# caoql98/LKGD

Measured on AMD Instinct MI355X. Metric: denoised frames/sec (14f x 576x1024, 25-step Euler), higher is better.
Workload: dtype f16; 1 GPU; SVD 14 frames x 576x1024, 25 Euler steps, CFG 1.0->3.0, single clip, vanilla pipeline_stable_video_diffusion_trans loop (configs[1]); unet=random-init SVD shapes (320,640,1280,1280), heads (5,10,20,20), 1.52 B params, parallelism=single GPU

## Files before the change

lkgd_amd/csrc/norm.hip:

```cpp
#include "common.h"
#include "../../include/lkgd_hip_dit.h"

static thread_local int gn_apply_kb = 32;
extern "C" void lkgd_debug_set_gn_apply_kb(int kb) { gn_apply_kb = kb < 32 ? 32 : kb; }
static thread_local int gn_stats_kb = 128;
extern "C" void lkgd_debug_set_gn_stats_kb(int kb) { gn_stats_kb = kb < 32 ? 32 : kb; }
static thread_local int gn_target_wgs = 1024;
extern "C" void lkgd_debug_set_gn_target_wgs(int n) { gn_target_wgs = n < 1 ? 1 : n; }
static inline int gn_rows_kb(int C, int kb, long long rows_per_sample, long long nsamples) {
  int rmax = kb * 1024 / (C * 2);
  rmax = rmax < 8 ? 8 : (rmax > 1024 ? 1024 : rmax);
  int rmin = 8 * 1024 / (C * 2);
  rmin = rmin < 8 ? 8 : rmin;
  if (rmin > rmax) rmin = rmax;
  const long long want = (rows_per_sample * nsamples + gn_target_wgs - 1) / gn_target_wgs;
  return (int)(want < rmin ? rmin : (want > rmax ? rmax : want));
}
static inline int gn_rows(int C, long long rows_per_sample, long long nsamples) {
  return gn_rows_kb(C, gn_apply_kb, rows_per_sample, nsamples);
}
static inline int gn_rows_stats(int C, long long rows_per_sample, long long nsamples) {
  return gn_rows_kb(C, gn_stats_kb, rows_per_sample, nsamples);
}
#define GN_GROUPS 32
#define GN_MAXC 4096

struct GnMap {
  int C8, rows_par, nslot;
};
__device__ __forceinline__ GnMap gn_map(int C) {
  GnMap m;
  m.C8 = C >> 3;
  if (m.C8 <= 256) { m.rows_par = 256 / m.C8; m.nslot = 1; }
  else { m.rows_par = 1; m.nslot = (m.C8 + 255) / 256; }
  return m;
}

__device__ __forceinline__ half8_t gn_load(const half_t* x0, int c0, int ld0, const half_t* x1, int ld1,
                                            long long row, int cv) {
  int c = cv << 3;
  if (c < c0) return *(const half8_t*)(x0 + row * ld0 + c);
  return *(const half8_t*)(x1 + row * ld1 + (c - c0));
}

__global__ __launch_bounds__(256) void gn_stats_kernel(const half_t* x0, int c0, int ld0, const half_t* x1, int c1,
                                                       int ld1, long long rows_per_sample, float* partial,
                                                       int nchunks, int GN_ROWS) {
  __shared__ float s_sum[GN_MAXC];
  __shared__ float s_sq[GN_MAXC];
  const int C = c0 + c1;
  const GnMap mp = gn_map(C);
  const int t = threadIdx.x;
  const int chunk = blockIdx.x;
  const long long sample = blockIdx.y;
  const long long r0 = (long long)chunk * GN_ROWS;
  long long r1 = r0 + GN_ROWS;
  if (r1 > rows_per_sample) r1 = rows_per_sample;
  const long long base = sample * rows_per_sample;
  for (int slot = 0; slot < mp.nslot; ++slot) {
    int cv, rp;
    if (mp.nslot == 1) { rp = t / mp.C8; cv = t - rp * mp.C8; if (rp >= mp.rows_par) continue; }
    else { rp = 0; cv = t + 256 * slot; if (cv >= mp.C8) continue; }
    float s[8], q[8];
#pragma unroll
    for (int e = 0; e < 8; ++e) { s[e] = 0.f; q[e] = 0.f; }
#pragma unroll 8
    for (long long r = r0 + rp; r < r1; r += mp.rows_par) {
      half8_t v = gn_load(x0, c0, ld0, x1, ld1, base + r, cv);
#pragma unroll
      for (int e = 0; e < 8; ++e) { float f = (float)v[e]; s[e] += f; q[e] += f * f; }
    }
#pragma unroll
    for (int e = 0; e < 8; ++e) {
      s_sum[rp * C + cv * 8 + e] = s[e];
      s_sq[rp * C + cv * 8 + e] = q[e];
    }
  }
  __syncthreads();
  if (t < GN_GROUPS) {
    const int gs = C / GN_GROUPS;
    float a = 0.f, b = 0.f;
    for (int rp = 0; rp < mp.rows_par; ++rp)
      for (int c = t * gs; c < (t + 1) * gs; ++c) { a += s_sum[rp * C + c]; b += s_sq[rp * C + c]; }
    float* o = partial + ((sample * nchunks + chunk) * GN_GROUPS + t) * 2;
    o[0] = a; o[1] = b;
  }
}

__device__ __forceinline__ void gn_reduce_pair(const float* partial, int nchunks, long long sample, int g, int lane,
                                               double& sa, double& sb) {
  double a = 0.0, b = 0.0;
  for (int c = lane; c < nchunks; c += 64) {
    const float* p = partial + ((sample * nchunks + c) * GN_GROUPS + g) * 2;
    a += p[0]; b += p[1];
  }
#pragma unroll
  for (int o = 32; o > 0; o >>= 1) { a += __shfl_xor(a, o, 64); b += __shfl_xor(b, o, 64); }
  sa = a; sb = b;
}

__global__ __launch_bounds__(256) void gn_finalize_kernel(const float* partial, int nchunks, double inv_count,
                                                          float eps, float* stats) {
  const int lane = threadIdx.x & 63;
  const int g = blockIdx.x * 4 + (threadIdx.x >> 6);
  const long long sample = blockIdx.y;
  double sa, sb;
  gn_reduce_pair(partial, nchunks, sample, g, lane, sa, sb);
  if (lane == 0) {
    double mean = sa * inv_count;
    double var = sb * inv_count - mean * mean;
    if (var < 0.0) var = 0.0;
    stats[(sample * GN_GROUPS + g) * 2 + 0] = (float)mean;
    stats[(sample * GN_GROUPS + g) * 2 + 1] = (float)(1.0 / sqrt(var + (double)eps));
  }
}

__global__ __launch_bounds__(256) void gn_cols_kernel(const float* cs0, int blk0, int ld0, int c0, const float* cs1, int blk1,
                                                      int ld1, int c1, long long rows_per_sample, double inv_count, float eps,
                                                      int as_sums, float* stats) {
  __shared__ double sa[256], sb[256];
  const int t = threadIdx.x;
  const int g = blockIdx.x;
  const long long sample = blockIdx.y;
  const int gs = (c0 + c1) / GN_GROUPS;
  double a = 0.0, b = 0.0;
  for (int src = 0; src < 2; ++src) {
    const float* cs = src ? cs1 : cs0;
    if (!cs) continue;
    const int blk = src ? blk1 : blk0, ld = src ? ld1 : ld0;
    int lo = g * gs - (src ? c0 : 0), hi = lo + gs;
    const int cmax = src ? c1 : c0;
    lo = lo < 0 ? 0 : lo;
    hi = hi > cmax ? cmax : hi;
    const int nch = hi - lo;
    if (nch <= 0) continue;
    const int plo = lo >> 1, npair = nch >> 1;
    const long long nb = rows_per_sample / blk, b0 = sample * nb;
    const long long total = nb * npair;
    for (long long e = t; e < total; e += 256) {
      const long long bi = e / npair;
      const int c = plo + (int)(e - bi * npair);
      const float* q = cs + ((b0 + bi) * (ld >> 1) + c) * 2;
      a += q[0]; b += q[1];
    }
  }
  sa[t] = a; sb[t] = b;
  __syncthreads();
#pragma unroll
  for (int o = 128; o > 0; o >>= 1) {
    if (t < o) { sa[t] += sa[t + o]; sb[t] += sb[t + o]; }
    __syncthreads();
  }
  if (t == 0) {
    float* o = stats + (sample * GN_GROUPS + g) * 2;
    if (as_sums) {
      o[0] = (float)sa[0]; o[1] = (float)sb[0];
    } else {
      const double mean = sa[0] * inv_count;
      double var = sb[0] * inv_count - mean * mean;
      if (var < 0.0) var = 0.0;
      o[0] = (float)mean;
      o[1] = (float)(1.0 / sqrt(var + (double)eps));
    }
  }
}

__global__ __launch_bounds__(256) void gn_sums_kernel(const float* partial, int nchunks, float* sums) {
  const int lane = threadIdx.x & 63;
  const int g = blockIdx.x * 4 + (threadIdx.x >> 6);
  const long long sample = blockIdx.y;
  double sa, sb;
  gn_reduce_pair(partial, nchunks, sample, g, lane, sa, sb);
  if (lane == 0) {
    sums[(sample * GN_GROUPS + g) * 2 + 0] = (float)sa;
    sums[(sample * GN_GROUPS + g) * 2 + 1] = (float)sb;
  }
}
__global__ void gn_finalize_sums_kernel(const float* sums, long long n, double inv_count, float eps, float* stats) {
  long long i = (long long)blockIdx.x * blockDim.x + threadIdx.x;
  if (i >= n) return;
  double mean = (double)sums[i * 2] * inv_count;
  double var = (double)sums[i * 2 + 1] * inv_count - mean * mean;
  if (var < 0.0) var = 0.0;
  stats[i * 2] = (float)mean;
  stats[i * 2 + 1] = (float)(1.0 / sqrt(var + (double)eps));
}

__global__ __launch_bounds__(256) void gn_apply_kernel(const half_t* x0, int c0, int ld0, const half_t* x1, int c1,
                                                       int ld1, long long rows_per_sample, const float* stats,
                                                       const float* gamma, const float* beta, int silu,
                                                       half_t* out, int ldo, int GN_ROWS) {
  const int C = c0 + c1;
  const GnMap mp = gn_map(C);
  const int t = threadIdx.x;
  const long long sample = blockIdx.y;
  const long long r0 = (long long)blockIdx.x * GN_ROWS;
  long long r1 = r0 + GN_ROWS;
  if (r1 > rows_per_sample) r1 = rows_per_sample;
  const long long base = sample * rows_per_sample;
  const int gs = C / GN_GROUPS;
  for (int slot = 0; slot < mp.nslot; ++slot) {
    int cv, rp;
    if (mp.nslot == 1) { rp = t / mp.C8; cv = t - rp * mp.C8; if (rp >= mp.rows_par) continue; }
    else { rp = 0; cv = t + 256 * slot; if (cv >= mp.C8) continue; }
    float A[8], B[8];
    {
      const float4_t g0 = *(const float4_t*)(gamma + cv * 8), g1 = *(const float4_t*)(gamma + cv * 8 + 4);
      const float4_t b0 = *(const float4_t*)(beta + cv * 8), b1 = *(const float4_t*)(beta + cv * 8 + 4);
      typedef float float2_t __attribute__((ext_vector_type(2)));
#pragma unroll
      for (int e = 0; e < 8; ++e) {
        const int g = (cv * 8 + e) / gs;
        const float2_t mr = *(const float2_t*)(stats + (sample * GN_GROUPS + g) * 2);
        const float ga = e < 4 ? g0[e & 3] : g1[e & 3], be = e < 4 ? b0[e & 3] : b1[e & 3];
        A[e] = mr[1] * ga;
        B[e] = be - mr[0] * A[e];
      }
    }
#pragma unroll 4
    for (long long r = r0 + rp; r < r1; r += mp.rows_par) {
      half8_t v = gn_load(x0, c0, ld0, x1, ld1, base + r, cv);
      half8_t o;
#pragma unroll
      for (int e = 0; e < 8; ++e) {
        float f = (float)v[e] * A[e] + B[e];
        if (silu) f = silu_f(f);
        o[e] = (half_t)f;
      }
      *(half8_t*)(out + (base + r) * ldo + cv * 8) = o;
    }
  }
}

static int gn_check(const void* x0, int c0, int ld0, const void* x1, int c1, int ld1, long long nsamples,
                    long long rows) {
  if (!x0) return LKGD_E_NULL;
  if (c1 > 0 && !x1) return LKGD_E_NULL;
  int C = c0 + c1;
  if (c0 <= 0 || c1 < 0 || C % GN_GROUPS || C % 8 || c0 % 8 || C > GN_MAXC) return LKGD_E_SHAPE;
  if (ld0 % 8 || (c1 > 0 && ld1 % 8)) return LKGD_E_ALIGN;
  if (!aligned16(x0) || (x1 && !aligned16(x1))) return LKGD_E_ALIGN;
  if (nsamples <= 0 || rows <= 0 || nsamples > 65535) return LKGD_E_SHAPE;
  return LKGD_OK;
}

extern "C" int lkgd_groupnorm_chunks(int64_t rows_per_sample, int32_t C) {
  const int ra = gn_rows(C, rows_per_sample, 1), rs = gn_rows_stats(C, rows_per_sample, 1);
  const int r = ra < rs ? ra : rs;
  return (int)((rows_per_sample + r - 1) / r);
}

extern "C" int lkgd_groupnorm_stats(const void* x0, int32_t c0, int32_t ld0, const void* x1, int32_t c1, int32_t ld1,
                                    int64_t nsamples, int64_t rows_per_sample, float eps, float* partial,
                                    float* stats, lkgd_stream_t stream) {
  int rc = gn_check(x0, c0, ld0, x1, c1, ld1, nsamples, rows_per_sample);
  if (rc) return rc;
  if (!partial || !stats) return LKGD_E_NULL;
  const int rs = gn_rows_stats(c0 + c1, rows_per_sample, nsamples);
  int nchunks = (int)((rows_per_sample + rs - 1) / rs);
  hipLaunchKernelGGL(gn_stats_kernel, dim3(nchunks, (unsigned)nsamples), dim3(256), 0, (hipStream_t)stream,
                     (const half_t*)x0, c0, ld0, (const half_t*)x1, c1, ld1, (long long)rows_per_sample, partial,
                     nchunks, rs);
  double inv = 1.0 / ((double)rows_per_sample * (double)((c0 + c1) / GN_GROUPS));
  hipLaunchKernelGGL(gn_finalize_kernel, dim3(8, (unsigned)nsamples), dim3(256), 0, (hipStream_t)stream, partial,
                     nchunks, inv, eps, stats);
  return hipGetLastError() == hipSuccess ? LKGD_OK : LKGD_E_LAUNCH;
}

extern "C" int lkgd_groupnorm_stats_cols(const float* cs0, int32_t blk0, int32_t ldcs0, int32_t c0, const float* cs1,
                                         int32_t blk1, int32_t ldcs1, int32_t c1, int64_t nsamples, int64_t rows_per_sample,
                                         float eps, int32_t as_sums, float* stats, lkgd_stream_t stream) {
  if (!cs0 || !stats || (c1 > 0 && !cs1)) return LKGD_E_NULL;
  const int C = c0 + c1;
  if ((C / GN_GROUPS) % 2 || c0 % 2 || c1 % 2 || ldcs0 % 2 || ldcs1 % 2) return LKGD_E_SHAPE;
  if (c0 <= 0 || c1 < 0 || C % GN_GROUPS || blk0 <= 0 || ldcs0 < c0 || (c1 > 0 && (blk1 <= 0 || ldcs1 < c1))) return LKGD_E_SHAPE;
  if (nsamples <= 0 || nsamples > 65535 || rows_per_sample <= 0 || rows_per_sample % blk0 || (c1 > 0 && rows_per_sample % blk1))
    return LKGD_E_SHAPE;
  const double inv = 1.0 / ((double)rows_per_sample * (double)(C / GN_GROUPS));
  hipLaunchKernelGGL(gn_cols_kernel, dim3(GN_GROUPS, (unsigned)nsamples), dim3(256), 0, (hipStream_t)stream, cs0, blk0, ldcs0,
                     c0, c1 > 0 ? cs1 : (const float*)nullptr, blk1, ldcs1, c1, (long long)rows_per_sample, inv, eps, as_sums,
                     stats);
  return hipGetLastError() == hipSuccess ? LKGD_OK : LKGD_E_LAUNCH;
}

extern "C" int lkgd_groupnorm_sums(const void* x0, int32_t c0, int32_t ld0, const void* x1, int32_t c1, int32_t ld1,
                                   int64_t nsamples, int64_t rows_per_sample, float* partial, float* sums,
                                   lkgd_stream_t stream) {
  int rc = gn_check(x0, c0, ld0, x1, c1, ld1, nsamples, rows_per_sample);
  if (rc) return rc;
  if (!partial || !sums) return LKGD_E_NULL;
  const int rs = gn_rows_stats(c0 + c1, rows_per_sample, nsamples);
  int nchunks = (int)((rows_per_sample + rs - 1) / rs);
  hipLaunchKernelGGL(gn_stats_kernel, dim3(nchunks, (unsigned)nsamples), dim3(256), 0, (hipStream_t)stream,
                     (const half_t*)x0, c0, ld0, (const half_t*)x1, c1, ld1, (long long)rows_per_sample, partial,
                     nchunks, rs);
  hipLaunchKernelGGL(gn_sums_kernel, dim3(8, (unsigned)nsamples), dim3(256), 0, (hipStream_t)stream, partial, nchunks,
                     sums);
  return hipGetLastError() == hipSuccess ? LKGD_OK : LKGD_E_LAUNCH;
}

__global__ void gn_finalize_parts_kernel(const float* parts, int nparts, long long part_stride, long long sample_stride,
                                         long long n, double inv_count, float eps, float* stats) {
  long long i = (long long)blockIdx.x * blockDim.x + threadIdx.x;
  if (i >= n) return;
  const long long sample = i / GN_GROUPS;
  const int g = (int)(i - sample * GN_GROUPS);
  double a = 0.0, b = 0.0;
  for (int r = 0; r < nparts; ++r) {
    const float* p = parts + r * part_stride + sample * sample_stride + g * 2;
    a += (double)p[0]; b += (double)p[1];
  }
  double mean = a * inv_count;
  double var = b * inv_count - mean * mean;
  if (var < 0.0) var = 0.0;
  stats[i * 2] = (float)mean;
  stats[i * 2 + 1] = (float)(1.0 / sqrt(var + (double)eps));
}

extern "C" int lkgd_groupnorm_finalize_parts(const float* parts, int32_t nparts, int64_t part_stride, int64_t nsamples,
                                             int64_t sample_stride, double count_per_group, float eps, float* stats,
                                             lkgd_stream_t stream) {
  if (!parts || !stats) return LKGD_E_NULL;
  if (nparts <= 0 || nsamples <= 0 || part_stride < 0 || sample_stride < GN_GROUPS * 2 || !(count_per_group > 0.0)) return LKGD_E_SHAPE;
  if (((uintptr_t)parts & 3u) != 0) return LKGD_E_ALIGN;
  long long n = nsamples * GN_GROUPS;
  hipLaunchKernelGGL(gn_finalize_parts_kernel, dim3((unsigned)((n + 255) / 256)), dim3(256), 0, (hipStream_t)stream, parts,
                     nparts, (long long)part_stride, (long long)sample_stride, n, 1.0 / count_per_group, eps, stats);
  return hipGetLastError() == hipSuccess ? LKGD_OK : LKGD_E_LAUNCH;
}

extern "C" int lkgd_groupnorm_finalize(const float* sums, int64_t nsamples, double count_per_group, float eps,
                                       float* stats, lkgd_stream_t stream) {
  if (!sums || !stats) return LKGD_E_NULL;
  if (nsamples <= 0 || !(count_per_group > 0.0)) return LKGD_E_SHAPE;
  long long n = nsamples * GN_GROUPS;
  hipLaunchKernelGGL(gn_finalize_sums_kernel, dim3((unsigned)((n + 255) / 256)), dim3(256), 0, (hipStream_t)stream,
                     sums, n, 1.0 / count_per_group, eps, stats);
  return hipGetLastError() == hipSuccess ? LKGD_OK : LKGD_E_LAUNCH;
}

extern "C" int lkgd_groupnorm_apply(const void* x0, int32_t c0, int32_t ld0, const void* x1, int32_t c1, int32_t ld1,
                                    int64_t nsamples, int64_t rows_per_sample, const float* stats,
                                    const float* gamma, const float* beta, int32_t silu, void* out, int32_t ldo,
                                    lkgd_stream_t stream) {
  int rc = gn_check(x0, c0, ld0, x1, c1, ld1, nsamples, rows_per_sample);
  if (rc) return rc;
  if (!stats || !gamma || !beta || !out) return LKGD_E_NULL;
  if (ldo % 8 || !aligned16(out)) return LKGD_E_ALIGN;
  const int ra = gn_rows(c0 + c1, rows_per_sample, nsamples);
  int nchunks = (int)((rows_per_sample + ra - 1) / ra);
  hipLaunchKernelGGL(gn_apply_kernel, dim3(nchunks, (unsigned)nsamples), dim3(256), 0, (hipStream_t)stream,
                     (const half_t*)x0, c0, ld0, (const half_t*)x1, c1, ld1, (long long)rows_per_sample, stats, gamma,
                     beta, silu, (half_t*)out, ldo, ra);
  return hipGetLastError() == hipSuccess ? LKGD_OK : LKGD_E_LAUNCH;
}

struct gn_segment { const half_t* src; half_t* dst; long long rows; long long sample; };
__global__ __launch_bounds__(256) void gn_apply_segments_kernel(const gn_segment* segs, int C, int ld, const float* stats,
                                                                const float* gamma, const float* beta, int silu, int GN_ROWS) {
  const gn_segment sg = segs[blockIdx.y];
  const long long r0 = (long long)blockIdx.x * GN_ROWS;
  if (r0 >= sg.rows) return;
  long long r1 = r0 + GN_ROWS;
  if (r1 > sg.rows) r1 = sg.rows;
  const GnMap mp = gn_map(C);
  const int t = threadIdx.x;
  const int gs = C / GN_GROUPS;
  for (int slot = 0; slot < mp.nslot; ++slot) {
    int cv, rp;
    if (mp.nslot == 1) { rp = t / mp.C8; cv = t - rp * mp.C8; if (rp >= mp.rows_par) continue; }
    else { rp = 0; cv = t + 256 * slot; if (cv >= mp.C8) continue; }
    float A[8], B[8];
    {
      const float4_t g0 = *(const float4_t*)(gamma + cv * 8), g1 = *(const float4_t*)(gamma + cv * 8 + 4);
      const float4_t b0 = *(const float4_t*)(beta + cv * 8), b1 = *(const float4_t*)(beta + cv * 8 + 4);
      typedef float float2_t __attribute__((ext_vector_type(2)));
#pragma unroll
      for (int e = 0; e < 8; ++e) {
        const int g = (cv * 8 + e) / gs;
        const float2_t mr = *(const float2_t*)(stats + (sg.sample * GN_GROUPS + g) * 2);
        const float ga = e < 4 ? g0[e & 3] : g1[e & 3], be = e < 4 ? b0[e & 3] : b1[e & 3];
        A[e] = mr[1] * ga;
        B[e] = be - mr[0] * A[e];
      }
    }
#pragma unroll 4
    for (long long r = r0 + rp; r < r1; r += mp.rows_par) {
      const half8_t v = *(const half8_t*)(sg.src + r * ld + cv * 8);
      half8_t o;
#pragma unroll
      for (int e = 0; e < 8; ++e) {
        float f = (float)v[e] * A[e] + B[e];
        if (silu) f = silu_f(f);
        o[e] = (half_t)f;
      }
      *(half8_t*)(sg.dst + r * ld + cv * 8) = o;
    }
  }
}

extern "C" int lkgd_groupnorm_apply_segments(const void* segs, int32_t nseg, int64_t max_rows, int32_t C, int32_t ld,
                                             const float* stats, const float* gamma, const float* beta, int32_t silu,
                                             lkgd_stream_t stream) {
  if (!segs || !stats || !gamma || !beta) return LKGD_E_NULL;
  if (nseg <= 0 || nseg > 65535 || max_rows <= 0 || C <= 0 || C % GN_GROUPS || C % 8 || C > GN_MAXC || ld % 8 || ld < C) return LKGD_E_SHAPE;
  if (((uintptr_t)segs & 7u) != 0) return LKGD_E_ALIGN;
  const int ra = gn_rows(C, max_rows, nseg);
  const int nchunks = (int)((max_rows + ra - 1) / ra);
  hipLaunchKernelGGL(gn_apply_segments_kernel, dim3(nchunks, (unsigned)nseg), dim3(256), 0, (hipStream_t)stream,
                     (const gn_segment*)segs, C, ld, stats, gamma, beta, silu, ra);
  return hipGetLastError() == hipSuccess ? LKGD_OK : LKGD_E_LAUNCH;
}

#define GN_SMALL_NT 512
#define GN_SMALL_U 4
template <int VEC>
__global__ __launch_bounds__(GN_SMALL_NT) void gn_small_kernel(const half_t* x0, int c0, int ld0, const half_t* x1, int c1, int ld1,
                                                               int rows, float eps, const float* gamma, const float* beta, int silu,
                                                               half_t* out, int ldo, float* stats) {
  typedef half_t hv_t __attribute__((ext_vector_type(VEC)));
  extern __shared__ __attribute__((aligned(16))) char gn_smem[];
  hv_t* buf = (hv_t*)gn_smem;
  __shared__ double red[2 * (GN_SMALL_NT / 64)];
  __shared__ float mr[2];
  const int t = threadIdx.x, lane = t & 63, w = t >> 6;
  const int g = blockIdx.x;
  const long long sample = blockIdx.y;
  const int gs = (c0 + c1) / GN_GROUPS, per = gs / VEC;
  const int units = rows * per;
  const long long base = sample * rows;
  const int q = GN_SMALL_NT / per, rem = GN_SMALL_NT - q * per;
  int r = t / per, a = t - r * per;
  float s = 0.f, ss = 0.f;
  for (int u = t; u < units; u += GN_SMALL_NT * GN_SMALL_U) {
    hv_t v[GN_SMALL_U];
#pragma unroll
    for (int k = 0; k < GN_SMALL_U; ++k) {
      const int c = g * gs + a * VEC;
      const bool ok = u + k * GN_SMALL_NT < units;
      const long long row = ok ? base + r : base;
      const half_t* src = c < c0 ? x0 + row * ld0 + c : x1 + row * ld1 + (c - c0);
      v[k] = *(const hv_t*)src;
      r += q; a += rem;
      if (a >= per) { a -= per; ++r; }
    }
#pragma unroll
    for (int k = 0; k < GN_SMALL_U; ++k) {
      if (u + k * GN_SMALL_NT < units) {
        buf[u + k * GN_SMALL_NT] = v[k];
#pragma unroll
        for (int e = 0; e < VEC; ++e) { const float f = (float)v[k][e]; s += f; ss += f * f; }
      }
    }
  }
#pragma unroll
  for (int o = 32; o > 0; o >>= 1) { s += __shfl_xor(s, o, 64); ss += __shfl_xor(ss, o, 64); }
  if (lane == 0) { red[w] = (double)s; red[GN_SMALL_NT / 64 + w] = (double)ss; }
  __syncthreads();
  if (t == 0) {
    const double inv = 1.0 / ((double)rows * (double)gs);
    double sa = 0.0, sb = 0.0;
#pragma unroll
    for (int i = 0; i < GN_SMALL_NT / 64; ++i) { sa += red[i]; sb += red[GN_SMALL_NT / 64 + i]; }
    const double mean = sa * inv;
    double var = sb * inv - mean * mean;
    if (var < 0.0) var = 0.0;
    mr[0] = (float)mean;
    mr[1] = (float)(1.0 / sqrt(var + (double)eps));
    if (stats) { stats[(sample * GN_GROUPS + g) * 2] = mr[0]; stats[(sample * GN_GROUPS + g) * 2 + 1] = mr[1]; }
  }
  __syncthreads();
  const float mean = mr[0], rstd = mr[1];
  r = t / per; a = t - r * per;
  for (int u = t; u < units; u += GN_SMALL_NT) {
    const int c = g * gs + a * VEC;
    const hv_t v = buf[u];
    hv_t o;
#pragma unroll
    for (int e = 0; e < VEC; ++e) {
      const float A = rstd * gamma[c + e], B = beta[c + e] - mean * A;
      float f = (float)v[e] * A + B;
      if (silu) f = silu_f(f);
      o[e] = (half_t)f;
    }
    *(hv_t*)(out + (base + r) * ldo + c) = o;
    r += q; a += rem;
    if (a >= per) { a -= per; ++r; }
  }
}

static thread_local int gn_small_on = 1;
extern "C" void lkgd_debug_set_gn_small(int on) { gn_small_on = on != 0; }
#define GN_SMALL_LDS (48 * 1024)
static thread_local long long gn_small_max_bytes = 10LL * 1024 * 1024 + 512 * 1024;
extern "C" void lkgd_debug_set_gn_small_limits(int64_t total_bytes) { gn_small_max_bytes = total_bytes; }
static int gn_small_vec(int c0, int c1, int ld0, int ld1, int ldo, long long nsamples, long long rows, const void* out) {
  const int C = c0 + c1, gs = C / GN_GROUPS;
  if (!gn_small_on || rows * gs * 2 > GN_SMALL_LDS || nsamples * rows * C * 2 > gn_small_max_bytes || nsamples * GN_GROUPS < 64)
    return 0;
  const int vec = gs % 8 == 0 ? 8 : (gs % 4 == 0 ? 4 : (gs % 2 == 0 ? 2 : 0));
  if (!vec || gs / vec > GN_SMALL_NT || c0 % vec || ld0 % vec || (c1 > 0 && ld1 % vec) || ldo % vec) return 0;
  if (((uintptr_t)out) % (2 * vec)) return 0;
  return vec;
}

extern "C" int lkgd_groupnorm_silu(const void* x0, int32_t c0, int32_t ld0, const void* x1, int32_t c1, int32_t ld1,
                                   int64_t nsamples, int64_t rows_per_sample, float eps, float* partial, float* stats,
                                   const float* gamma, const float* beta, int32_t silu, void* out, int32_t ldo,
                                   lkgd_stream_t stream) {
  const int vec = gn_small_vec(c0, c1, ld0, ld1, ldo, nsamples, rows_per_sample, out);
  if (vec) {
    int rc = gn_check(x0, c0, ld0, x1, c1, ld1, nsamples, rows_per_sample);
    if (rc) return rc;
    if (!gamma || !beta || !out) return LKGD_E_NULL;
    LKGD_DEVICE_ONCE_BEGIN
      if (hipFuncSetAttribute((const void*)gn_small_kernel<8>, hipFuncAttributeMaxDynamicSharedMemorySize, GN_SMALL_LDS) != hipSuccess ||
          hipFuncSetAttribute((const void*)gn_small_kernel<4>, hipFuncAttributeMaxDynamicSharedMemorySize, GN_SMALL_LDS) != hipSuccess ||
          hipFuncSetAttribute((const void*)gn_small_kernel<2>, hipFuncAttributeMaxDynamicSharedMemorySize, GN_SMALL_LDS) != hipSuccess)
        return LKGD_E_LAUNCH;
    LKGD_DEVICE_ONCE_END
    const size_t lds = (size_t)rows_per_sample * ((c0 + c1) / GN_GROUPS) * 2;
    const dim3 grid(GN_GROUPS, (unsigned)nsamples);
#define GN_SMALL_GO(V)                                                                                                   \
  hipLaunchKernelGGL(gn_small_kernel<V>, grid, dim3(GN_SMALL_NT), lds, (hipStream_t)stream, (const half_t*)x0, c0, ld0,          \
                     (const half_t*)x1, c1, ld1, (int)rows_per_sample, eps, gamma, beta, silu, (half_t*)out, ldo, stats)
    if (vec == 8) GN_SMALL_GO(8); else if (vec == 4) GN_SMALL_GO(4); else GN_SMALL_GO(2);
#undef GN_SMALL_GO
    return hipGetLastError() == hipSuccess ? LKGD_OK : LKGD_E_LAUNCH;
  }
  int rc = lkgd_groupnorm_stats(x0, c0, ld0, x1, c1, ld1, nsamples, rows_per_sample, eps, partial, stats, stream);
  if (rc) return rc;
  return lkgd_groupnorm_apply(x0, c0, ld0, x1, c1, ld1, nsamples, rows_per_sample, stats, gamma, beta, silu, out, ldo, stream);
}

#define LN_MAXV 3
#define LN_MAXV_WIDE 4
#define LN_MAXV_XWIDE 6
template <int L, bool AFF, int NV = LN_MAXV>
__global__ __launch_bounds__(256) void layernorm_kernel(const half_t* x, int ldx, long long T, int C,
                                                        const float* gamma, const float* beta, float eps,
                                                        const half_t* rowbias, int ldrb, int d1, int m1, int d2,
                                                        int md, int c0, half_t* out, int ldo) {
  constexpr int RPW = 64 / L;
  const int lane = threadIdx.x & 63;
  const int wave = threadIdx.x >> 6;
  const int sub = lane / L, li = lane % L;
  const int C8 = C >> 3;
  float g[AFF ? NV : 1][8], b[AFF ? NV : 1][8];
  if (AFF) {
#pragma unroll
    for (int v = 0; v < NV; ++v) {
      int cv = li + L * v;
      if (cv >= C8) cv = C8 - 1;
      const float4_t g0 = *(const float4_t*)(gamma + cv * 8), g1 = *(const float4_t*)(gamma + cv * 8 + 4);
      const float4_t b0 = *(const float4_t*)(beta + cv * 8), b1 = *(const float4_t*)(beta + cv * 8 + 4);
#pragma unroll
      for (int e = 0; e < 8; ++e) {
        g[AFF ? v : 0][e] = e < 4 ? g0[e & 3] : g1[e & 3];
        b[AFF ? v : 0][e] = e < 4 ? b0[e & 3] : b1[e & 3];
      }
    }
  }
  const float invC = 1.0f / (float)C;
  const long long rows_per_block = 4 * RPW;
  for (long long row0 = (long long)blockIdx.x * rows_per_block + wave * RPW; row0 < T;
       row0 += (long long)gridDim.x * rows_per_block) {
    const long long row = row0 + sub;
    const bool live = row < T;
    float xv[NV][8];
    float s = 0.f;
    long long idx = 0;
    if (rowbias && live) {
      if (T < (1LL << 31)) {
        const unsigned ru = (unsigned)row;
        idx = ((ru / (unsigned)d1) * (unsigned)m1 + (ru % (unsigned)d2) + (unsigned)c0) % (unsigned)md;
      } else {
        idx = ((row / d1) * m1 + (row % d2) + c0) % md;
      }
    }
#pragma unroll
    for (int v = 0; v < NV; ++v) {
      int cv = li + L * v;
      if (live && cv < C8) {
        half8_t h = *(const half8_t*)(x + row * ldx + cv * 8);
        if (rowbias) {
          half8_t rb = *(const half8_t*)(rowbias + idx * ldrb + cv * 8);
          h = h + rb;
        }
#pragma unroll
        for (int e = 0; e < 8; ++e) { xv[v][e] = (float)h[e]; s += xv[v][e]; }
      } else {
#pragma unroll
        for (int e = 0; e < 8; ++e) xv[v][e] = 0.f;
      }
    }
#pragma unroll
    for (int o = L / 2; o > 0; o >>= 1) s += __shfl_xor(s, o, 64);
    const float mean = s * invC;
    float q = 0.f;
#pragma unroll
    for (int v = 0; v < NV; ++v) {
      int cv = li + L * v;
      if (cv < C8) {
#pragma unroll
        for (int e = 0; e < 8; ++e) { float d = xv[v][e] - mean; q += d * d; }
      }
    }
#pragma unroll
    for (int o = L / 2; o > 0; o >>= 1) q += __shfl_xor(q, o, 64);
    const float rstd = rsqrtf(q * invC + eps);
#pragma unroll
    for (int v = 0; v < NV; ++v) {
      int cv = li + L * v;
      if (live && cv < C8) {
        half8_t o;
#pragma unroll
        for (int e = 0; e < 8; ++e) {
          float y = (xv[v][e] - mean) * rstd;
          if (AFF) y = y * g[AFF ? v : 0][e] + b[AFF ? v : 0][e];
          o[e] = (half_t)y;
        }
        *(half8_t*)(out + row * ldo + cv * 8) = o;
      }
    }
  }
}

extern "C" int lkgd_layernorm(const void* x, int32_t ldx, int64_t T, int32_t C, const float* gamma,
                              const float* beta, float eps, const void* rowbias, int32_t ldrb, int32_t rb_d1,
                              int32_t rb_m1, int32_t rb_d2, int32_t rb_md, void* out, int32_t ldo,
                              lkgd_stream_t stream) {
  if (!x || !out) return LKGD_E_NULL;
  if ((gamma == nullptr) != (beta == nullptr)) return LKGD_E_NULL;
  if (T <= 0 || C <= 0 || C % 8 || C > 64 * 8 * LN_MAXV_XWIDE) return LKGD_E_SHAPE;
  if (ldx % 8 || ldo % 8 || !aligned16(x) || !aligned16(out)) return LKGD_E_ALIGN;
  if (rowbias && (ldrb % 8 || !aligned16(rowbias) || rb_d1 <= 0 || rb_d2 <= 0 || rb_md <= 0)) return LKGD_E_SHAPE;
  const int C8 = C / 8;
  int L = 4;
  while (L < 64 && L * LN_MAXV < C8) L *= 2;
  const long long rows_per_block = 4 * (64 / L);
  long long blocks = (T + rows_per_block - 1) / rows_per_block;
  if (blocks > 256 * 16) blocks = 256 * 16;
#define LN_LAUNCH(LL)                                                                                            \
  if (gamma)                                                                                                     \
    hipLaunchKernelGGL((layernorm_kernel<LL, true>), dim3((unsigned)blocks), dim3(256), 0, (hipStream_t)stream,  \
                       (const half_t*)x, ldx, (long long)T, C, gamma, beta, eps, (const half_t*)rowbias, ldrb,   \
                       rb_d1, rb_m1, rb_d2, rb_md, 0, (half_t*)out, ldo);                                        \
  else                                                                                                           \
    hipLaunchKernelGGL((layernorm_kernel<LL, false>), dim3((unsigned)blocks), dim3(256), 0, (hipStream_t)stream, \
                       (const half_t*)x, ldx, (long long)T, C, gamma, beta, eps, (const half_t*)rowbias, ldrb,   \
                       rb_d1, rb_m1, rb_d2, rb_md, 0, (half_t*)out, ldo)
  if (C8 > 64 * LN_MAXV_WIDE) {
    if (gamma)
      hipLaunchKernelGGL((layernorm_kernel<64, true, LN_MAXV_XWIDE>), dim3((unsigned)blocks), dim3(256), 0, (hipStream_t)stream,
                         (const half_t*)x, ldx, (long long)T, C, gamma, beta, eps, (const half_t*)rowbias, ldrb, rb_d1, rb_m1,
                         rb_d2, rb_md, 0, (half_t*)out, ldo);
    else
      hipLaunchKernelGGL((layernorm_kernel<64, false, LN_MAXV_XWIDE>), dim3((unsigned)blocks), dim3(256), 0, (hipStream_t)stream,
                         (const half_t*)x, ldx, (long long)T, C, gamma, beta, eps, (const half_t*)rowbias, ldrb, rb_d1, rb_m1,
                         rb_d2, rb_md, 0, (half_t*)out, ldo);
    return hipGetLastError() == hipSuccess ? LKGD_OK : LKGD_E_LAUNCH;
  }
  if (C8 > 64 * LN_MAXV) {
    if (gamma)
      hipLaunchKernelGGL((layernorm_kernel<64, true, LN_MAXV_WIDE>), dim3((unsigned)blocks), dim3(256), 0, (hipStream_t)stream,
                         (const half_t*)x, ldx, (long long)T, C, gamma, beta, eps, (const half_t*)rowbias, ldrb, rb_d1, rb_m1,
                         rb_d2, rb_md, 0, (half_t*)out, ldo);
    else
      hipLaunchKernelGGL((layernorm_kernel<64, false, LN_MAXV_WIDE>), dim3((unsigned)blocks), dim3(256), 0, (hipStream_t)stream,
                         (const half_t*)x, ldx, (long long)T, C, gamma, beta, eps, (const half_t*)rowbias, ldrb, rb_d1, rb_m1,
                         rb_d2, rb_md, 0, (half_t*)out, ldo);
    return hipGetLastError() == hipSuccess ? LKGD_OK : LKGD_E_LAUNCH;
  }
  switch (L) {
    case 4: LN_LAUNCH(4); break;
    case 8: LN_LAUNCH(8); break;
    case 16: LN_LAUNCH(16); break;
    case 32: LN_LAUNCH(32); break;
    default: LN_LAUNCH(64); break;
  }
#undef LN_LAUNCH
  return hipGetLastError() == hipSuccess ? LKGD_OK : LKGD_E_LAUNCH;
}

__device__ __forceinline__ half8_t qk_rope8(half8_t x, const float* __restrict__ cs, const float* __restrict__ sn) {
#pragma clang fp contract(off)
  half8_t y;
#pragma unroll
  for (int i = 0; i < 4; ++i) {
    const float a = (float)x[2 * i], b = (float)x[2 * i + 1];
    const float pa = a * cs[2 * i], pb = b * sn[2 * i];
    const float qa = b * cs[2 * i + 1], qb = a * sn[2 * i + 1];
    y[2 * i] = (half_t)(pa - pb);
    y[2 * i + 1] = (half_t)(qa + qb);
  }
  return y;
}

__device__ __forceinline__ void qk_norm_rope_head(half_t* __restrict__ p, bool live, const half8_t (&hv)[2],
                                                  const float (&g)[2][8], const float (&b)[2][8], float eps, bool rot,
                                                  const float (&cs)[2][8], const float (&sn)[2][8]) {
  const float invC = 1.0f / 64.0f;
  float xv[2][8];
  float s = 0.f;
#pragma unroll
  for (int v = 0; v < 2; ++v) {
    if (live) {
#pragma unroll
      for (int e = 0; e < 8; ++e) { xv[v][e] = (float)hv[v][e]; s += xv[v][e]; }
    } else {
#pragma unroll
      for (int e = 0; e < 8; ++e) xv[v][e] = 0.f;
    }
  }
#pragma unroll
  for (int o = 2; o > 0; o >>= 1) s += __shfl_xor(s, o, 64);
  const float mean = s * invC;
  float q = 0.f;
#pragma unroll
  for (int v = 0; v < 2; ++v) {
#pragma unroll
    for (int e = 0; e < 8; ++e) { float d = xv[v][e] - mean; q += d * d; }
  }
#pragma unroll
  for (int o = 2; o > 0; o >>= 1) q += __shfl_xor(q, o, 64);
  const float rstd = rsqrtf(q * invC + eps);
#pragma unroll
  for (int v = 0; v < 2; ++v) {
    if (live) {
      half8_t o;
#pragma unroll
      for (int e = 0; e < 8; ++e) {
        float y = (xv[v][e] - mean) * rstd;
        y = y * g[v][e] + b[v][e];
        o[e] = (half_t)y;
      }
      if (rot) o = qk_rope8(o, cs[v], sn[v]);
      *(half8_t*)(p + 32 * v) = o;
    }
  }
}

__global__ __launch_bounds__(256) void qk_norm_rope_kernel(half_t* q, int ldq, half_t* k, int ldk, long long rows, int heads,
                                                           const float* __restrict__ gamma_q, const float* __restrict__ beta_q,
                                                           const float* __restrict__ gamma_k, const float* __restrict__ beta_k,
                                                           float eps, const float* __restrict__ cos_t,
                                                           const float* __restrict__ sin_t, int ldt, int rows_per_batch,
                                                           int split) {
  const int lane = threadIdx.x & 63;
  const int wave = threadIdx.x >> 6;
  const int sub = lane >> 2, li = lane & 3;
  float gq[2][8], bq[2][8], gk[2][8], bk[2][8];
#pragma unroll
  for (int v = 0; v < 2; ++v) {
    const int c = (li + 4 * v) * 8;
#pragma unroll
    for (int e = 0; e < 8; e += 4) {
      const float4_t a0 = *(const float4_t*)(gamma_q + c + e), a1 = *(const float4_t*)(beta_q + c + e);
      const float4_t a2 = *(const float4_t*)(gamma_k + c + e), a3 = *(const float4_t*)(beta_k + c + e);
#pragma unroll
      for (int j = 0; j < 4; ++j) { gq[v][e + j] = a0[j]; bq[v][e + j] = a1[j]; gk[v][e + j] = a2[j]; bk[v][e + j] = a3[j]; }
    }
  }
  for (long long tok = (long long)blockIdx.x * 4 + wave; tok < rows; tok += (long long)gridDim.x * 4) {
    const int r = rows < (1LL << 31) ? (int)((unsigned)tok % (unsigned)rows_per_batch) : (int)(tok % rows_per_batch);
    const bool rot = cos_t != nullptr && r >= split;
    float cs[2][8], sn[2][8];
#pragma unroll
    for (int v = 0; v < 2; ++v) {
#pragma unroll
      for (int e = 0; e < 8; ++e) { cs[v][e] = 1.f; sn[v][e] = 0.f; }
      if (rot) {
        const long long t0 = (long long)(r - split) * ldt + (li + 4 * v) * 8;
#pragma unroll
        for (int e = 0; e < 8; e += 4) {
          const float4_t c4 = *(const float4_t*)(cos_t + t0 + e), s4 = *(const float4_t*)(sin_t + t0 + e);
#pragma unroll
          for (int j = 0; j < 4; ++j) { cs[v][e + j] = c4[j]; sn[v][e + j] = s4[j]; }
        }
      }
    }
    for (int h0 = 0; h0 < heads; h0 += 16) {
      const int h = h0 + sub;
      const bool live = h < heads;
      half_t* pq = q + tok * ldq + h * 64 + li * 8;
      half_t* pk = k + tok * ldk + h * 64 + li * 8;
      half8_t hq[2], hk[2];
      if (live) {
#pragma unroll
        for (int v = 0; v < 2; ++v) { hq[v] = *(const half8_t*)(pq + 32 * v); hk[v] = *(const half8_t*)(pk + 32 * v); }
      }
      qk_norm_rope_head(pq, live, hq, gq, bq, eps, rot, cs, sn);
      qk_norm_rope_head(pk, live, hk, gk, bk, eps, rot, cs, sn);
    }
  }
}

extern "C" int lkgd_qk_norm_rope(void* q, int32_t ldq, void* k, int32_t ldk, int64_t rows, int32_t heads,
                                 const float* gamma_q, const float* beta_q, const float* gamma_k, const float* beta_k,
                                 float eps, const float* cos_t, const float* sin_t, int32_t ldt, int32_t rows_per_batch,
                                 int32_t split, lkgd_stream_t stream) {
  if (!q || !k || !gamma_q || !beta_q || !gamma_k || !beta_k) return LKGD_E_NULL;
  if ((cos_t == nullptr) != (sin_t == nullptr)) return LKGD_E_NULL;
  if (rows <= 0 || heads <= 0 || rows_per_batch <= 0 || rows % rows_per_batch || split < 0 || split > rows_per_batch)
    return LKGD_E_SHAPE;
  if ((long long)heads * 64 > ldq || (long long)heads * 64 > ldk) return LKGD_E_SHAPE;
  if (cos_t && ldt < 64) return LKGD_E_SHAPE;
  if (ldq % 8 || ldk % 8 || !aligned16(q) || !aligned16(k) || !aligned16(gamma_q) || !aligned16(beta_q) ||
      !aligned16(gamma_k) || !aligned16(beta_k))
    return LKGD_E_ALIGN;
  if (cos_t && (ldt % 4 || !aligned16(cos_t) || !aligned16(sin_t))) return LKGD_E_ALIGN;
  long long blocks = (rows + 3) / 4;
  if (blocks > 256 * 16) blocks = 256 * 16;
  hipLaunchKernelGGL(qk_norm_rope_kernel, dim3((unsigned)blocks), dim3(256), 0, (hipStream_t)stream, (half_t*)q, ldq,
                     (half_t*)k, ldk, (long long)rows, heads, gamma_q, beta_q, gamma_k, beta_k, eps, cos_t, sin_t, ldt,
                     rows_per_batch, split);
  return hipGetLastError() == hipSuccess ? LKGD_OK : LKGD_E_LAUNCH;
}
```

Baseline: 6.080 frames/s.

## Rework GroupNorm stats/apply kernels: adaptive block size, register group reduction, prefetched rows

The GroupNorm stats kernel drops the per-channel shared-memory arrays. Each thread now folds its 8 channels into group partial sums in registers and writes them to a compact dynamic LDS buffer, and a parallel 8-lanes-per-group shuffle reduction replaces the serial 32-thread tail. Block size is now picked per channel count (256, 320 or a multiple of 64) so threads map evenly onto C/8 vectors, which removes the multi-slot loop. The apply kernels use a templated SILU branch with two-deep software prefetch of rows, and the stats loop issues four loads per iteration. This adds template variants and debug macros, and block sizes that are not powers of two may change occupancy.

Result: no change. 6.084 frames/s (median of 6 runs) (+0.1%).

```diff
diff --git a/lkgd_amd/csrc/norm.hip b/lkgd_amd/csrc/norm.hip
--- a/lkgd_amd/csrc/norm.hip
+++ b/lkgd_amd/csrc/norm.hip
@@ -24,67 +24,134 @@
 }
 #define GN_GROUPS 32
 #define GN_MAXC 4096
-
+#ifdef LKGD_X_GN_NOSILU
+#define GN_SILU(f) (f)
+#else
+#define GN_SILU(f) silu_f(f)
+#endif
+
+#define GN_MAX_THREADS 512
+static inline int gn_threads(int C) {
+  const int C8 = C >> 3;
+  if (C8 > 320) return (C8 + 63) / 64 * 64;
+  return (320 / C8) * C8 * 256 > (256 / C8) * C8 * 320 ? 320 : 256;
+}
 struct GnMap {
-  int C8, rows_par, nslot;
+  int C8, rows_par, rp, cv;
+  bool on;
 };
 __device__ __forceinline__ GnMap gn_map(int C) {
   GnMap m;
   m.C8 = C >> 3;
-  if (m.C8 <= 256) { m.rows_par = 256 / m.C8; m.nslot = 1; }
-  else { m.rows_par = 1; m.nslot = (m.C8 + 255) / 256; }
+  m.rows_par = (int)blockDim.x / m.C8;
+  m.rp = (int)threadIdx.x / m.C8;
+  m.cv = (int)threadIdx.x - m.rp * m.C8;
+  m.on = m.rp < m.rows_par;
   return m;
 }
 
-__device__ __forceinline__ half8_t gn_load(const half_t* x0, int c0, int ld0, const half_t* x1, int ld1,
-                                            long long row, int cv) {
-  int c = cv << 3;
-  if (c < c0) return *(const half8_t*)(x0 + row * ld0 + c);
-  return *(const half8_t*)(x1 + row * ld1 + (c - c0));
-}
-
-__global__ __launch_bounds__(256) void gn_stats_kernel(const half_t* x0, int c0, int ld0, const half_t* x1, int c1,
-                                                       int ld1, long long rows_per_sample, float* partial,
-                                                       int nchunks, int GN_ROWS) {
-  __shared__ float s_sum[GN_MAXC];
-  __shared__ float s_sq[GN_MAXC];
+struct GnSrc {
+  const half_t* p;
+  long long ld;
+};
+__device__ __forceinline__ GnSrc gn_src(const half_t* x0, int c0, int ld0, const half_t* x1, int ld1, int cv) {
+  const int c = cv << 3;
+  GnSrc s;
+  if (c < c0) { s.p = x0 + c; s.ld = ld0; }
+  else { s.p = x1 + (c - c0); s.ld = ld1; }
+  return s;
+}
+
+template <int KMAX>
+__global__ __launch_bounds__(GN_MAX_THREADS) void gn_stats_kernel(const half_t* x0, int c0, int ld0, const half_t* x1, int c1,
+                                                                  int ld1, long long rows_per_sample, float* partial,
+                                                                  int nchunks, int GN_ROWS) {
+  extern __shared__ __attribute__((aligned(16))) char gn_stats_smem[];
+  float2_t* seg = (float2_t*)gn_stats_smem;
   const int C = c0 + c1;
   const GnMap mp = gn_map(C);
-  const int t = threadIdx.x;
+  const int t = threadIdx.x, nt = blockDim.x;
   const int chunk = blockIdx.x;
   const long long sample = blockIdx.y;
+  const int gs = C / GN_GROUPS;
   const long long r0 = (long long)chunk * GN_ROWS;
   long long r1 = r0 + GN_ROWS;
   if (r1 > rows_per_sample) r1 = rows_per_sample;
-  const long long base = sample * rows_per_sample;
-  for (int slot = 0; slot < mp.nslot; ++slot) {
-    int cv, rp;
-    if (mp.nslot == 1) { rp = t / mp.C8; cv = t - rp * mp.C8; if (rp >= mp.rows_par) continue; }
-    else { rp = 0; cv = t + 256 * slot; if (cv >= mp.C8) continue; }
+  if (mp.on) {
     float s[8], q[8];
 #pragma unroll
     for (int e = 0; e < 8; ++e) { s[e] = 0.f; q[e] = 0.f; }
-#pragma unroll 8
-    for (long long r = r0 + rp; r < r1; r += mp.rows_par) {
-      half8_t v = gn_load(x0, c0, ld0, x1, ld1, base + r, cv);
-#pragma unroll
-      for (int e = 0; e < 8; ++e) { float f = (float)v[e]; s[e] += f; q[e] += f * f; }
-    }
+    const GnSrc src = gn_src(x0, c0, ld0, x1, ld1, mp.cv);
+    const half_t* p = src.p + (sample * rows_per_sample + r0 + mp.rp) * src.ld;
+    const long long step = mp.rows_par * src.ld;
+    const int n = (int)(r1 - r0);
+    for (int i = mp.rp; i < n; i += 4 * mp.rows_par, p += 4 * step) {
+      half8_t v[4];
+#pragma unroll
+      for (int k = 0; k < 4; ++k) {
+        v[k] = (half8_t)((half_t)0);
+        if (i + k * mp.rows_par < n) v[k] = *(const half8_t*)(p + k * step);
+      }
+#pragma unroll
+      for (int k = 0; k < 4; ++k) {
+#pragma unroll
+        for (int e = 0; e < 8; ++e) { float f = (float)v[k][e]; s[e] += f; q[e] += f * f; }
+      }
+    }
+#ifdef LKGD_X_GN_NOTAIL
+    float fold = 0.f;
+#pragma unroll
+    for (int e = 0; e < 8; ++e) fold += s[e] + q[e];
+    if (fold == 12345.678f) partial[0] = fold;
+#else
+    const int c = mp.cv << 3, g0 = c / gs, nlo = (g0 + 1) * gs - c;
+    float2_t acc[KMAX];
+#pragma unroll
+    for (int k = 0; k < KMAX; ++k) acc[k] = (float2_t)(0.f);
 #pragma unroll
     for (int e = 0; e < 8; ++e) {
-      s_sum[rp * C + cv * 8 + e] = s[e];
-      s_sq[rp * C + cv * 8 + e] = q[e];
-    }
-  }
+      const int k = KMAX == 2 ? (e >= nlo ? 1 : 0) : (c + e) / gs - g0;
+#pragma unroll
+      for (int kk = 0; kk < KMAX; ++kk) {
+        acc[kk].x += k == kk ? s[e] : 0.f;
+        acc[kk].y += k == kk ? q[e] : 0.f;
+      }
+    }
+#pragma unroll
+    for (int k = 0; k < KMAX; ++k) seg[k * nt + mp.cv * mp.rows_par + mp.rp] = acc[k];
+#endif
+  }
+#ifndef LKGD_X_GN_NOTAIL
   __syncthreads();
-  if (t < GN_GROUPS) {
-    const int gs = C / GN_GROUPS;
+  if (t < GN_GROUPS * 8) {
+    const int g = t >> 3, j = t & 7;
     float a = 0.f, b = 0.f;
-    for (int rp = 0; rp < mp.rows_par; ++rp)
-      for (int c = t * gs; c < (t + 1) * gs; ++c) { a += s_sum[rp * C + c]; b += s_sq[rp * C + c]; }
-    float* o = partial + ((sample * nchunks + chunk) * GN_GROUPS + t) * 2;
-    o[0] = a; o[1] = b;
-  }
+#pragma unroll
+    for (int k = 0; k < KMAX; ++k) {
+      const int gg = g - k;
+      if (gg < 0 || (k > 0 && KMAX == 2 && (gs & 7) == 0)) continue;
+      const int lo = ((gg * gs + 7) >> 3) * mp.rows_par, hi = (((gg + 1) * gs + 7) >> 3) * mp.rows_par;
+      for (int i = lo + j; i < hi; i += 8) { const float2_t v = seg[k * nt + i]; a += v.x; b += v.y; }
+    }
+#pragma unroll
+    for (int o = 1; o < 8; o <<= 1) { a += __shfl_xor(a, o, 64); b += __shfl_xor(b, o, 64); }
+    if (j == 0) {
+      float* o = partial + ((sample * nchunks + chunk) * GN_GROUPS + g) * 2;
+      o[0] = a; o[1] = b;
+    }
+  }
+#endif
+}
+static void gn_stats_launch(const void* x0, int c0, int ld0, const void* x1, int c1, int ld1, long long nsamples,
+                            long long rows_per_sample, float* partial, int nchunks, int rs, hipStream_t stream) {
+  const int C = c0 + c1, nt = gn_threads(C);
+  const dim3 grid(nchunks, (unsigned)nsamples);
+  if (C / GN_GROUPS >= 8)
+    hipLaunchKernelGGL(gn_stats_kernel<2>, grid, dim3(nt), 2 * nt * sizeof(float2_t), stream, (const half_t*)x0, c0, ld0,
+                       (const half_t*)x1, c1, ld1, rows_per_sample, partial, nchunks, rs);
+  else
+    hipLaunchKernelGGL(gn_stats_kernel<8>, grid, dim3(nt), 8 * nt * sizeof(float2_t), stream, (const half_t*)x0, c0, ld0,
+                       (const half_t*)x1, c1, ld1, rows_per_sample, partial, nchunks, rs);
 }
 
 __device__ __forceinline__ void gn_reduce_pair(const float* partial, int nchunks, long long sample, int g, int lane,
@@ -186,50 +253,71 @@
   stats[i * 2 + 1] = (float)(1.0 / sqrt(var + (double)eps));
 }
 
-__global__ __launch_bounds__(256) void gn_apply_kernel(const half_t* x0, int c0, int ld0, const half_t* x1, int c1,
-                                                       int ld1, long long rows_per_sample, const float* stats,
-                                                       const float* gamma, const float* beta, int silu,
-                                                       half_t* out, int ldo, int GN_ROWS) {
+__device__ __forceinline__ void gn_scale_shift(const float* stats, long long sample, const float* gamma, const float* beta,
+                                               int cv, int gs, float (&A)[8], float (&B)[8]) {
+  const float4_t g0 = *(const float4_t*)(gamma + cv * 8), g1 = *(const float4_t*)(gamma + cv * 8 + 4);
+  const float4_t b0 = *(const float4_t*)(beta + cv * 8), b1 = *(const float4_t*)(beta + cv * 8 + 4);
+#pragma unroll
+  for (int e = 0; e < 8; ++e) {
+    const int g = (cv * 8 + e) / gs;
+    const float2_t mr = *(const float2_t*)(stats + (sample * GN_GROUPS + g) * 2);
+    const float ga = e < 4 ? g0[e & 3] : g1[e & 3], be = e < 4 ? b0[e & 3] : b1[e & 3];
+    A[e] = mr[1] * ga;
+    B[e] = be - mr[0] * A[e];
+  }
+}
+#define GN_NB 2
+template <bool SILU>
+__device__ __forceinline__ void gn_apply_rows(const half_t* src, long long lds, half_t* dst, long long ldd, int i, int n,
+                                              int step, const float (&A)[8], const float (&B)[8]) {
+  if (i >= n) return;
+  src += i * lds;
+  dst += i * ldd;
+  const long long sstep = step * lds, dstep = step * ldd;
+  const half_t* const first = src;
+  half8_t v[GN_NB], nv[GN_NB];
+#pragma unroll
+  for (int k = 0; k < GN_NB; ++k) v[k] = *(const half8_t*)(i + k * step < n ? src + k * sstep : first);
+  for (; i < n; i += GN_NB * step, dst += GN_NB * dstep) {
+    src += GN_NB * sstep;
+#pragma unroll
+    for (int k = 0; k < GN_NB; ++k) nv[k] = *(const half8_t*)(i + (GN_NB + k) * step < n ? src + k * sstep : first);
+#pragma unroll
+    for (int k = 0; k < GN_NB; ++k) {
+      if (i + k * step < n) {
+        half8_t o;
+#pragma unroll
+        for (int e = 0; e < 8; ++e) {
+          float f = (float)v[k][e] * A[e] + B[e];
+          if (SILU) f = GN_SILU(f);
+          o[e] = (half_t)f;
+        }
+        *(half8_t*)(dst + k * dstep) = o;
+      }
+      v[k] = nv[k];
+    }
+  }
+}
+
+__global__ __launch_bounds__(GN_MAX_THREADS) void gn_apply_kernel(const half_t* x0, int c0, int ld0, const half_t* x1, int c1,
+                                                                  int ld1, long long rows_per_sample, const float* stats,
+                                                                  const float* gamma, const float* beta, int silu,
+                                                                  half_t* out, int ldo, int GN_ROWS) {
   const int C = c0 + c1;
   const GnMap mp = gn_map(C);
-  const int t = threadIdx.x;
+  if (!mp.on) return;
   const long long sample = blockIdx.y;
   const long long r0 = (long long)blockIdx.x * GN_ROWS;
   long long r1 = r0 + GN_ROWS;
   if (r1 > rows_per_sample) r1 = rows_per_sample;
   const long long base = sample * rows_per_sample;
-  const int gs = C / GN_GROUPS;
-  for (int slot = 0; slot < mp.nslot; ++slot) {
-    int cv, rp;
-    if (mp.nslot == 1) { rp = t / mp.C8; cv = t - rp * mp.C8; if (rp >= mp.rows_par) continue; }
-    else { rp = 0; cv = t + 256 * slot; if (cv >= mp.C8) continue; }
-    float A[8], B[8];
-    {
-      const float4_t g0 = *(const float4_t*)(gamma + cv * 8), g1 = *(const float4_t*)(gamma + cv * 8 + 4);
-      const float4_t b0 = *(const float4_t*)(beta + cv * 8), b1 = *(const float4_t*)(beta + cv * 8 + 4);
-      typedef float float2_t __attribute__((ext_vector_type(2)));
-#pragma unroll
-      for (int e = 0; e < 8; ++e) {
-        const int g = (cv * 8 + e) / gs;
-        const float2_t mr = *(const float2_t*)(stats + (sample * GN_GROUPS + g) * 2);
-        const float ga = e < 4 ? g0[e & 3] : g1[e & 3], be = e < 4 ? b0[e & 3] : b1[e & 3];
-        A[e] = mr[1] * ga;
-        B[e] = be - mr[0] * A[e];
-      }
-    }
-#pragma unroll 4
-    for (long long r = r0 + rp; r < r1; r += mp.rows_par) {
-      half8_t v = gn_load(x0, c0, ld0, x1, ld1, base + r, cv);
-      half8_t o;
-#pragma unroll
-      for (int e = 0; e < 8; ++e) {
-        float f = (float)v[e] * A[e] + B[e];
-        if (silu) f = silu_f(f);
-        o[e] = (half_t)f;
-      }
-      *(half8_t*)(out + (base + r) * ldo + cv * 8) = o;
-    }
-  }
+  float A[8], B[8];
+  gn_scale_shift(stats, sample, gamma, beta, mp.cv, C / GN_GROUPS, A, B);
+  const GnSrc src = gn_src(x0, c0, ld0, x1, ld1, mp.cv);
+  const half_t* sp = src.p + (base + r0) * src.ld;
+  half_t* dp = out + (base + r0) * ldo + mp.cv * 8;
+  if (silu) gn_apply_rows<true>(sp, src.ld, dp, ldo, mp.rp, (int)(r1 - r0), mp.rows_par, A, B);
+  else gn_apply_rows<false>(sp, src.ld, dp, ldo, mp.rp, (int)(r1 - r0), mp.rows_par, A, B);
 }
 
 static int gn_check(const void* x0, int c0, int ld0, const void* x1, int c1, int ld1, long long nsamples,
@@ -258,9 +346,7 @@
   if (!partial || !stats) return LKGD_E_NULL;
   const int rs = gn_rows_stats(c0 + c1, rows_per_sample, nsamples);
   int nchunks = (int)((rows_per_sample + rs - 1) / rs);
-  hipLaunchKernelGGL(gn_stats_kernel, dim3(nchunks, (unsigned)nsamples), dim3(256), 0, (hipStream_t)stream,
-                     (const half_t*)x0, c0, ld0, (const half_t*)x1, c1, ld1, (long long)rows_per_sample, partial,
-                     nchunks, rs);
+  gn_stats_launch(x0, c0, ld0, x1, c1, ld1, nsamples, rows_per_sample, partial, nchunks, rs, (hipStream_t)stream);
   double inv = 1.0 / ((double)rows_per_sample * (double)((c0 + c1) / GN_GROUPS));
   hipLaunchKernelGGL(gn_finalize_kernel, dim3(8, (unsigned)nsamples), dim3(256), 0, (hipStream_t)stream, partial,
                      nchunks, inv, eps, stats);
@@ -291,9 +377,7 @@
   if (!partial || !sums) return LKGD_E_NULL;
   const int rs = gn_rows_stats(c0 + c1, rows_per_sample, nsamples);
   int nchunks = (int)((rows_per_sample + rs - 1) / rs);
-  hipLaunchKernelGGL(gn_stats_kernel, dim3(nchunks, (unsigned)nsamples), dim3(256), 0, (hipStream_t)stream,
-                     (const half_t*)x0, c0, ld0, (const half_t*)x1, c1, ld1, (long long)rows_per_sample, partial,
-                     nchunks, rs);
+  gn_stats_launch(x0, c0, ld0, x1, c1, ld1, nsamples, rows_per_sample, partial, nchunks, rs, (hipStream_t)stream);
   hipLaunchKernelGGL(gn_sums_kernel, dim3(8, (unsigned)nsamples), dim3(256), 0, (hipStream_t)stream, partial, nchunks,
                      sums);
   return hipGetLastError() == hipSuccess ? LKGD_OK : LKGD_E_LAUNCH;
@@ -349,54 +433,29 @@
   if (ldo % 8 || !aligned16(out)) return LKGD_E_ALIGN;
   const int ra = gn_rows(c0 + c1, rows_per_sample, nsamples);
   int nchunks = (int)((rows_per_sample + ra - 1) / ra);
-  hipLaunchKernelGGL(gn_apply_kernel, dim3(nchunks, (unsigned)nsamples), dim3(256), 0, (hipStream_t)stream,
+  hipLaunchKernelGGL(gn_apply_kernel, dim3(nchunks, (unsigned)nsamples), dim3(gn_threads(c0 + c1)), 0, (hipStream_t)stream,
                      (const half_t*)x0, c0, ld0, (const half_t*)x1, c1, ld1, (long long)rows_per_sample, stats, gamma,
                      beta, silu, (half_t*)out, ldo, ra);
   return hipGetLastError() == hipSuccess ? LKGD_OK : LKGD_E_LAUNCH;
 }
 
 struct gn_segment { const half_t* src; half_t* dst; long long rows; long long sample; };
-__global__ __launch_bounds__(256) void gn_apply_segments_kernel(const gn_segment* segs, int C, int ld, const float* stats,
-                                                                const float* gamma, const float* beta, int silu, int GN_ROWS) {
+__global__ __launch_bounds__(GN_MAX_THREADS) void gn_apply_segments_kernel(const gn_segment* segs, int C, int ld,
+                                                                           const float* stats, const float* gamma,
+                                                                           const float* beta, int silu, int GN_ROWS) {
   const gn_segment sg = segs[blockIdx.y];
   const long long r0 = (long long)blockIdx.x * GN_ROWS;
   if (r0 >= sg.rows) return;
   long long r1 = r0 + GN_ROWS;
   if (r1 > sg.rows) r1 = sg.rows;
   const GnMap mp = gn_map(C);
-  const int t = threadIdx.x;
-  const int gs = C / GN_GROUPS;
-  for (int slot = 0; slot < mp.nslot; ++slot) {
-    int cv, rp;
-    if (mp.nslot == 1) { rp = t / mp.C8; cv = t - rp * mp.C8; if (rp >= mp.rows_par) continue; }
-    else { rp = 0; cv = t + 256 * slot; if (cv >= mp.C8) continue; }
-    float A[8], B[8];
-    {
-      const float4_t g0 = *(const float4_t*)(gamma + cv * 8), g1 = *(const float4_t*)(gamma + cv * 8 + 4);
-      const float4_t b0 = *(const float4_t*)(beta + cv * 8), b1 = *(const float4_t*)(beta + cv * 8 + 4);
-      typedef float float2_t __attribute__((ext_vector_type(2)));
-#pragma unroll
-      for (int e = 0; e < 8; ++e) {
-        const int g = (cv * 8 + e) / gs;
-        const float2_t mr = *(const float2_t*)(stats + (sg.sample * GN_GROUPS + g) * 2);
-        const float ga = e < 4 ? g0[e & 3] : g1[e & 3], be = e < 4 ? b0[e & 3] : b1[e & 3];
-        A[e] = mr[1] * ga;
-        B[e] = be - mr[0] * A[e];
-      }
-    }
-#pragma unroll 4
-    for (long long r = r0 + rp; r < r1; r += mp.rows_par) {
-      const half8_t v = *(const half8_t*)(sg.src + r * ld + cv * 8);
-      half8_t o;
-#pragma unroll
-      for (int e = 0; e < 8; ++e) {
-        float f = (float)v[e] * A[e] + B[e];
-        if (silu) f = silu_f(f);
-        o[e] = (half_t)f;
-      }
-      *(half8_t*)(sg.dst + r * ld + cv * 8) = o;
-    }
-  }
+  if (!mp.on) return;
+  float A[8], B[8];
+  gn_scale_shift(stats, sg.sample, gamma, beta, mp.cv, C / GN_GROUPS, A, B);
+  const half_t* sp = sg.src + r0 * ld + mp.cv * 8;
+  half_t* dp = sg.dst + r0 * ld + mp.cv * 8;
+  if (silu) gn_apply_rows<true>(sp, ld, dp, ld, mp.rp, (int)(r1 - r0), mp.rows_par, A, B);
+  else gn_apply_rows<false>(sp, ld, dp, ld, mp.rp, (int)(r1 - r0), mp.rows_par, A, B);
 }
 
 extern "C" int lkgd_groupnorm_apply_segments(const void* segs, int32_t nseg, int64_t max_rows, int32_t C, int32_t ld,
@@ -407,7 +466,7 @@
   if (((uintptr_t)segs & 7u) != 0) return LKGD_E_ALIGN;
   const int ra = gn_rows(C, max_rows, nseg);
   const int nchunks = (int)((max_rows + ra - 1) / ra);
-  hipLaunchKernelGGL(gn_apply_segments_kernel, dim3(nchunks, (unsigned)nseg), dim3(256), 0, (hipStream_t)stream,
+  hipLaunchKernelGGL(gn_apply_segments_kernel, dim3(nchunks, (unsigned)nseg), dim3(gn_threads(C)), 0, (hipStream_t)stream,
                      (const gn_segment*)segs, C, ld, stats, gamma, beta, silu, ra);
   return hipGetLastError() == hipSuccess ? LKGD_OK : LKGD_E_LAUNCH;
 }
@@ -480,7 +539,7 @@
     for (int e = 0; e < VEC; ++e) {
       const float A = rstd * gamma[c + e], B = beta[c + e] - mean * A;
       float f = (float)v[e] * A + B;
-      if (silu) f = silu_f(f);
+      if (silu) f = GN_SILU(f);
       o[e] = (half_t)f;
     }
     *(hv_t*)(out + (base + r) * ldo + c) = o;
```
